# VachaLab/gorder

Hardware: AMD Instinct MI355X
Metric: trajectory frames/sec (higher is better)
Workload: dtype f32

## Files before the change

### gorder_amd/csrc/trajectory_driver.h

```cpp
#pragma once

#include <atomic>
#include <chrono>
#include <condition_variable>
#include <deque>
#include <mutex>
#include <thread>

#include "../../include/gorder_xtc.h"

namespace {

struct TrajSlot {
    float *h_xyz = nullptr, *h_box = nullptr, *h_time = nullptr;
    float *d_xyz = nullptr, *d_box = nullptr;
    uint8_t *h_blob = nullptr, *d_blob = nullptr;
    gorder_xtc_frame_t *h_frames = nullptr, *d_frames = nullptr;
    float *d_box_in = nullptr;
    uint32_t *d_stat = nullptr, *d_short = nullptr, *h_stat = nullptr, *h_short = nullptr;
    XtcCheckpoint *d_cp = nullptr;
    std::vector<int64_t> file_pos;
    std::vector<uint32_t> file_idx;
    uint32_t prefix_q16 = 65536;
    uint32_t kinds = 0;
    size_t moved = 0;
    uint64_t blob_bytes = 0;
    hipStream_t stream = nullptr;
    hipEvent_t staged = nullptr, copied = nullptr, computed = nullptr;
    bool copy_issued = false, compute_issued = false;
    uint32_t n = 0;
    std::vector<uint64_t> fidx;
};

struct TrajCache {
    static constexpr int kSlots = 4;
    TrajSlot slot[kSlots];
    bool dev = false, has_xtc = false;
    uint32_t batch = 0, n_stop = 0;
    size_t blob_cap = 0, xyz_bytes = 0;
    hipStream_t copy_stream = nullptr;
    unsigned long long *h_err = nullptr;
    float *h_fix = nullptr;
};

struct TrajPipe {
    static constexpr int kSlots = TrajCache::kSlots;
    TrajSlot *slot = nullptr;
    std::mutex mu;
    std::condition_variable cv;
    std::deque<int> free_q, filled_q;
    bool reader_done = false, stop = false;
    int reader_status = GORDER_XTC_OK;
    std::string reader_msg;
    double decode_s = 0.0, reader_stalled_s = 0.0, setup_s = 0.0;
    std::atomic<uint32_t> prefix_q16{65536};
    uint32_t reports = 0;
    bool alloc_failed = false;
};

double seconds_since(std::chrono::steady_clock::time_point t0) {
    return std::chrono::duration<double>(std::chrono::steady_clock::now() - t0).count();
}

void traj_cache_free(gorder_hip_handle *h) {
    TrajCache *c = static_cast<TrajCache *>(h->traj_cache);
    if (!c) return;
    for (TrajSlot &s : c->slot) {
        if (s.h_xyz) (void)hipHostFree(s.h_xyz);
        if (s.h_box) (void)hipHostFree(s.h_box);
        if (s.h_time) (void)hipHostFree(s.h_time);
        if (s.h_blob) (void)hipHostFree(s.h_blob);
        if (s.h_frames) (void)hipHostFree(s.h_frames);
        (void)hipFree(s.d_xyz);
        (void)hipFree(s.d_box);
        (void)hipFree(s.d_blob);
        (void)hipFree(s.d_frames);
        (void)hipFree(s.d_box_in);
        (void)hipFree(s.d_stat);
        (void)hipFree(s.d_short);
        (void)hipFree(s.d_cp);
        if (s.h_stat) (void)hipHostFree(s.h_stat);
        if (s.h_short) (void)hipHostFree(s.h_short);
        if (s.stream) (void)hipStreamDestroy(s.stream);
        if (s.staged) (void)hipEventDestroy(s.staged);
// ... 219 lines not shown
            {
                std::lock_guard<std::mutex> lk(pipe.mu);
                if (pipe.stop) return;
            }
            const auto t0 = std::chrono::steady_clock::now();
            const hipError_t e = alloc_slot(pipe.slot[k]);
            std::lock_guard<std::mutex> lk(pipe.mu);
            pipe.setup_s += seconds_since(t0);
            if (e != hipSuccess) { pipe.alloc_failed = true; return; }
            pipe.free_q.push_back(k);
            pipe.cv.notify_all();
        }
    });
    const double setup_s = seconds_since(t_start);

    gorder_xtc_pool *pool = nullptr;
    if (dev && gorder_xtc_pool_create(n_threads, &pool) != GORDER_XTC_OK) pool = nullptr;
    const char *forced_prefix = getenv("GORDER_HIP_PREFIX_Q16");
    const bool adapt_prefix = dev && has_xtc && !forced_prefix && !env_flag("GORDER_HIP_NO_PREFIX") && n_stop < n_file_atoms;
    if (dev && forced_prefix) pipe.prefix_q16.store((uint32_t)std::max(1l, std::min(65536l, atol(forced_prefix))));
    const bool verify = dev && has_xtc && (adapt_prefix || forced_prefix);
    const int device = h->device;
    std::thread reader([&, device]() {
        (void)hipSetDevice(device);
        uint64_t state = 0, analysed = shard_lo;
        double last_time = -INFINITY;
        uint32_t f = 0;
        gorder_xtc_reader *r = nullptr;
        bool done = shard_n == 0;
        uint32_t n_filled = 0;
        uint64_t to_skip = shard_lo, left = shard_n;
        auto give_up = [&](int st, const std::string &msg) {
            std::lock_guard<std::mutex> lk(pipe.mu);
            pipe.reader_status = st;
            pipe.reader_msg = msg;
            done = true;
        };
        while (!done) {
            int k = -1;
            {
                const auto t0 = std::chrono::steady_clock::now();
                std::unique_lock<std::mutex> lk(pipe.mu);
                pipe.cv.wait(lk, [&] { return pipe.stop || !pipe.free_q.empty(); });
                pipe.reader_stalled_s += seconds_since(t0);
                if (pipe.stop) break;
                k = pipe.free_q.front();
                pipe.free_q.pop_front();
            }
            TrajSlot &s = pipe.slot[k];
            const auto t_wait = std::chrono::steady_clock::now();
            if (s.copy_issued) (void)hipEventSynchronize(s.staged);
            const auto t1 = std::chrono::steady_clock::now();
            {
                std::lock_guard<std::mutex> lk(pipe.mu);
                pipe.reader_stalled_s += std::chrono::duration<double>(t1 - t_wait).count();
            }
            s.n = 0;
            s.blob_bytes = 0;
            uint32_t fill = batch;
            if (adapt_prefix && tr->batch_frames == 0 && f < tr->n_paths && file_is_xtc[f]) {
                if (n_filled == 0) fill = std::min(batch, 256u);
                else if (n_filled == 1) fill = std::min(batch, 1024u);
                else if (n_filled == 2) {
                    std::unique_lock<std::mutex> lk(pipe.mu);
                    pipe.cv.wait(lk, [&] { return pipe.stop || pipe.reports > 0; });
                }
            }
            s.prefix_q16 = pipe.prefix_q16.load();
            while (!done && s.n < fill) {
                if (left == 0) { done = true; break; }
                if (!r) {
                    if (f == tr->n_paths) { done = true; break; }
                    int st = gorder_xtc_open(tr->paths[f], tr->group, tr->n_group, &r);
                    if (st == GORDER_XTC_OK && gorder_xtc_n_atoms_out(r) != n_atoms) st = GORDER_XTC_ERR_ARGUMENT;
                    if (st != GORDER_XTC_OK) {
                        give_up(st, std::string("cannot read ") + tr->paths[f] +
                                        (st == GORDER_XTC_ERR_ARGUMENT ? ": atoms per frame differ from the tables" : ""));
                        break;
                    }
                }
                if (to_skip) {
                    const int64_t sk = gorder_xtc_skip_window(r, tr->begin_ps, tr->end_ps, tr->step, &state, &last_time, to_skip);
                    if (sk < 0) { give_up((int)sk, std::string("read error in ") + tr->paths[f]); break; }
                    to_skip -= (uint64_t)sk;
                    if (to_skip) {
                        gorder_xtc_close(r);
                        r = nullptr;
                        f++;
                        continue;
                    }
                }
                const uint64_t want = std::min<uint64_t>(fill - s.n, left);
                uint64_t used = 0;
                const int64_t got =
                    dev ? gorder_xtc_pack_window_ex(r, tr->begin_ps, tr->end_ps, tr->step, &state, &last_time,
                                                    s.h_blob + s.blob_bytes, blob_cap - s.blob_bytes, &used, s.h_frames + s.n,
                                                    s.h_box + 9u * (size_t)s.n, s.h_time + s.n, want, n_threads, pool,
                                                    s.prefix_q16, s.file_pos.data() + s.n)
                        : gorder_xtc_read_window_mt(r, tr->begin_ps, tr->end_ps, tr->step, &state, &last_time,
                                                    s.h_xyz + (size_t)s.n * n_atoms * 3u, s.h_box + 9u * (size_t)s.n,
                                                    s.h_time + s.n, want, n_threads);
                if (dev && got == GORDER_XTC_ERR_NO_SPACE) {
                    if (s.n > 0) break;
                    give_up(GORDER_XTC_ERR_ARGUMENT, std::string("a single frame of ") + tr->paths[f] + " does not fit the staging blob");
                    break;
                }
                if (got < 0) {
                    give_up((int)got, std::string("read error in ") + tr->paths[f]);
                    break;
                }
                if (got == 0) {
                    gorder_xtc_close(r);
                    r = nullptr;
                    f++;
                    continue;
                }
                if (dev) {
                    for (int64_t q = 0; q < got; q++) {
                        s.h_frames[s.n + (size_t)q].offset += s.blob_bytes;
                        s.file_idx[s.n + (size_t)q] = f;
                    }
                    s.blob_bytes += used;
                }
                s.n += (uint32_t)got;
                left -= (uint64_t)got;
            }
            if (pool) {
                const int cst = gorder_xtc_pool_wait(pool);
                if (cst != GORDER_XTC_OK && !done) give_up(cst, "read error while copying the compressed blocks");
                else if (cst != GORDER_XTC_OK) { std::lock_guard<std::mutex> lk(pipe.mu); if (pipe.reader_status == GORDER_XTC_OK) { pipe.reader_status = cst; pipe.reader_msg = "read error while copying the compressed blocks"; } }
            }
            const double dt = seconds_since(t1);
            std::lock_guard<std::mutex> lk(pipe.mu);
            pipe.decode_s += dt;
            if (s.n == 0 || pipe.reader_status != GORDER_XTC_OK) {
                pipe.free_q.push_front(k);
                break;
            }
            if (dev && (xtc_table_kinds(s.h_frames, s.n) & kXtcTableXtc)) n_filled++;
            s.fidx.resize((size_t)s.n);
            for (uint32_t q = 0; q < s.n; q++) s.fidx[q] = tr->first_frame_index + (analysed + q) * tr->step;
            analysed += s.n;
            pipe.filled_q.push_back(k);
            pipe.cv.notify_all();
        }
        if (r) gorder_xtc_close(r);
        std::lock_guard<std::mutex> lk(pipe.mu);
        pipe.reader_done = true;
        pipe.cv.notify_all();
    });

    int status = GORDER_OK;
    uint64_t frames = 0, batches = 0, bytes = 0, frames_fixed = 0;
    double starved_s = 0.0;
    std::string hip_msg;
    uint32_t need_q16 = 0;
    auto stage_a = [&](int k) {
        TrajSlot &s = pipe.slot[k];
        const size_t nx = (size_t)s.n * n_atoms * 3u * sizeof(float), nb = (size_t)s.n * 9u * sizeof(float);
        hipError_t e = hipSuccess;
        const hipStream_t feed = dev ? s.stream : copy_stream;
        if (s.compute_issued && !dev) e = hipStreamWaitEvent(feed, s.computed, 0);
        s.moved = nb;
        if (dev) {
            const size_t nf = (size_t)s.n * sizeof(gorder_xtc_frame_t);
            s.moved += (size_t)s.blob_bytes + nf;
            if (e == hipSuccess) e = hipMemsetAsync(s.d_stat, 0, 2 * sizeof(uint32_t), feed);
            if (e == hipSuccess) e = hipMemsetAsync(s.d_stat + 2, 0xff, 2 * sizeof(uint32_t), feed);
            if (e == hipSuccess) e = hipMemcpyAsync(s.d_blob, s.h_blob, (size_t)s.blob_bytes, hipMemcpyHostToDevice, feed);
            if (e == hipSuccess) e = hipMemcpyAsync(s.d_frames, s.h_frames, nf, hipMemcpyHostToDevice, feed);
            if (e == hipSuccess) e = hipMemcpyAsync(s.d_box_in, s.h_box, nb, hipMemcpyHostToDevice, feed);
            if (e == hipSuccess) e = hipEventRecord(s.staged, feed);
            if (e == hipSuccess && s.compute_issued) e = hipStreamWaitEvent(feed, s.computed, 0);
            if (e == hipSuccess) e = hipMemcpyAsync(s.d_box, s.d_box_in, nb, hipMemcpyDeviceToDevice, feed);
            s.kinds = xtc_table_kinds(s.h_frames, s.n);
            if (e == hipSuccess && status == GORDER_OK)
                status = xtc_decode_on(h, feed, s.d_blob, s.blob_bytes, s.d_frames, s.n, n_file_atoms, d_slot_of, n_stop,
// ... 91 lines not shown
            while (!pipe.filled_q.empty()) {
                fresh.push_back(pipe.filled_q.front());
                pipe.filled_q.pop_front();
            }
            finished = pipe.reader_done && fresh.empty() && decoding.empty();
        }
        if (finished) break;
        for (int k : fresh) {
            if (!go) break;
            stage_a(k);
            if (verify) decoding.push_back(k);
            else go = stage_b(k);
        }
        bool any = !fresh.empty();
        while (go && !decoding.empty() &&
               (status != GORDER_OK || hipEventQuery(pipe.slot[decoding.front()].copied) == hipSuccess)) {
            const int front = decoding.front();
            decoding.pop_front();
            go = stage_b(front);
            any = true;
        }
        if (go && !any && !decoding.empty()) {
            std::unique_lock<std::mutex> lk(pipe.mu);
            pipe.cv.wait_for(lk, std::chrono::microseconds(100), [&] { return !pipe.filled_q.empty(); });
        }
    }
    {
        std::lock_guard<std::mutex> lk(pipe.mu);
        pipe.stop = true;
        pipe.cv.notify_all();
    }
    reader.join();
    allocator.join();
    if (pool) gorder_xtc_pool_destroy(pool);
    (void)hipStreamSynchronize(copy_stream);
    for (int k = 0; k < TrajPipe::kSlots; k++)
        if (pipe.slot[k].stream) (void)hipStreamSynchronize(pipe.slot[k].stream);
    const int sync_status = gorder_hip_synchronize(h);
    if (status == GORDER_OK) status = sync_status;
    else if (!hip_msg.empty()) h->err_msg = hip_msg;
    if (status == GORDER_OK && pipe.reader_status != GORDER_XTC_OK) {
        status = pipe.reader_status == GORDER_XTC_ERR_FORMAT ? GORDER_ERR_TRAJECTORY_FORMAT : GORDER_ERR_INVALID_ARGUMENT;
        h->err_msg = pipe.reader_msg + " (reader status " + std::to_string(pipe.reader_status) + ")";
    }
    if (stats) {
        stats->n_frames = frames;
        stats->n_batches = batches;
        stats->bytes_h2d = bytes;
        stats->seconds_total = seconds_since(t_start);
        stats->seconds_decode = pipe.decode_s;
        stats->seconds_reader_stalled = pipe.reader_stalled_s;
        stats->seconds_gpu_starved = starved_s;
        stats->batch_frames = batch;
        stats->decoder_threads = n_threads;
        stats->device_decode = dev ? 1u : 0u;
        stats->frames_decoded_by_host = (uint32_t)std::min<uint64_t>(frames_fixed, UINT32_MAX);
        stats->seconds_setup = setup_s + pipe.setup_s;
        stats->shard_first = shard_lo;
        stats->shard_frames_total = tr->shard_count > 1 ? shard_total : frames;
    }
    cleanup();
    if (pipe.alloc_failed) traj_cache_free(h);
#undef TRAJ_TRY
    return status;
}
```

### gorder_amd/csrc/xtc_reader.cpp

```cpp
#include <algorithm>
#include <climits>
#include <cmath>
#include <cstdint>
#include <cstdio>
#include <cstring>
#include <string>
#include <string>
#include <atomic>
#include <chrono>
#include <condition_variable>
#include <deque>
#include <functional>
#include <memory>
#include <mutex>
#include <thread>
#include <immintrin.h>
#include <sys/mman.h>
#include <sys/stat.h>
#include <unistd.h>
#include <vector>

#include "../../include/gorder_xtc.h"

namespace {

const int kMagicInts[] = {
    0,       0,       0,       0,       0,       0,       0,       0,       0,       8,        10,       12,
    16,      20,      25,      32,      40,      50,      64,      80,      101,     128,      161,      203,
    256,     322,     406,     512,     645,     812,     1024,    1290,    1625,    2048,     2580,     3250,
    4096,    5060,    6501,    8192,    10321,   13003,   16384,   20642,   26007,   32768,    41285,    52015,
    65536,   82570,   104031,  131072,  165140,  208063,  262144,  330280,  416127,  524287,   660561,   832255,
    1048576, 1321122, 1664510, 2097152, 2642245, 3329021, 4194304, 5284491, 6658042, 8388607,  10568983, 13316085,
    16777216};
constexpr int kFirstIdx = 9;
constexpr int kLastIdx = (int)(sizeof(kMagicInts) / sizeof(kMagicInts[0]));

struct BitReader {
    const uint8_t *p;
    size_t n, bitpos = 0;
    bool overrun = false;

    static uint64_t load_be64(const uint8_t *q) {
        uint64_t w;
        memcpy(&w, q, 8);
        return __builtin_bswap64(w);
    }
    uint64_t bits57(int nbits) {
        if (nbits == 0) return 0;
// ... 104 lines not shown
    memcpy(&f, &u, 4);
    return f;
}

double bed(const uint8_t *p) {
    uint64_t u = 0;
    for (int k = 0; k < 8; k++) u = (u << 8) | p[k];
    double d;
    memcpy(&d, &u, 8);
    return d;
}

}

struct FileMap {
    const uint8_t *base = nullptr;
    size_t size = 0;
    ~FileMap() { if (base) munmap(const_cast<uint8_t *>(base), size); }
};

struct gorder_xtc_reader {
    std::string path;
    FILE *fp = nullptr;
    bool trr = false;
    bool gro = false;
    uint32_t natoms = 0;
    std::vector<uint32_t> group;
    std::vector<int32_t> slot_of;
    uint32_t n_needed = 0;
    std::vector<uint8_t> buf;
    std::vector<int> ints;
    std::shared_ptr<struct FileMap> map;
    bool map_tried = false;
};

namespace {

bool read_exact(FILE *fp, void *dst, size_t n) { return fread(dst, 1, n, fp) == n; }

int decode_ints(gorder_xtc_reader *r, const int minint[3], const int maxint[3], int smallidx, const uint8_t *data,
                size_t nbytes) {
    const uint32_t natoms = r->natoms;
    r->ints.resize((size_t)natoms * 3);
    uint32_t sizeint[3];
    int bitsizeint[3] = {0, 0, 0};
    for (int k = 0; k < 3; k++) {
        const int64_t s = (int64_t)maxint[k] - (int64_t)minint[k] + 1;
        if (s <= 0 || s > 0xffffffffll) return GORDER_XTC_ERR_FORMAT;
        sizeint[k] = (uint32_t)s;
    }
    int bitsize;
    if ((sizeint[0] | sizeint[1] | sizeint[2]) > 0xffffff) {
        for (int k = 0; k < 3; k++) bitsizeint[k] = size_of_int(sizeint[k]);
        bitsize = 0;
    } else {
        bitsize = size_of_ints(sizeint);
    }
    if (smallidx < kFirstIdx || smallidx >= kLastIdx) return GORDER_XTC_ERR_FORMAT;
    int smaller = kMagicInts[smallidx > kFirstIdx ? smallidx - 1 : kFirstIdx] / 2;
    int smallnum = kMagicInts[smallidx] / 2;
    uint32_t sizesmall[3] = {(uint32_t)kMagicInts[smallidx], (uint32_t)kMagicInts[smallidx], (uint32_t)kMagicInts[smallidx]};
    const uint64_t recip_big[3] = {reciprocal_of(sizeint[0]), reciprocal_of(sizeint[1]), reciprocal_of(sizeint[2])};
    uint64_t recip_small[3] = {kMagicRecips.r[smallidx], kMagicRecips.r[smallidx], kMagicRecips.r[smallidx]};

    BitReader br{data, nbytes};
    int *out = r->ints.data();
// ... 619 lines not shown
        *last_time = (double)t;
        if (t < begin_ps) continue;
        if (end_ps >= 0.0f && t > end_ps) { fseek(r->fp, 0, SEEK_END); break; }
        const uint64_t k = (*state)++;
        if (k % step != 0) continue;
        offsets.push_back(pos);
    }
    const size_t nout = gorder_xtc_n_atoms_out(r), n = offsets.size();
    const uint32_t nt = (uint32_t)std::min<size_t>(n_threads, std::max<size_t>(n, 1));
    std::vector<int> status(nt, GORDER_XTC_OK);
    std::vector<std::thread> pool;
    for (uint32_t w = 0; w < nt; w++)
        pool.emplace_back([&, w]() {
            gorder_xtc_reader *mine = nullptr;
            int st = gorder_xtc_open(r->path.c_str(), r->group.empty() ? nullptr : r->group.data(), (uint32_t)r->group.size(), &mine);
            for (size_t i = w; st == GORDER_XTC_OK && i < n; i += nt) {
                if (fseek(mine->fp, offsets[i], SEEK_SET) != 0) { st = GORDER_XTC_ERR_FORMAT; break; }
                float t = 0.0f;
                st = gorder_xtc_next(mine, xyz + i * nout * 3, box9 + i * 9, nullptr, &t, nullptr);
                if (st == GORDER_XTC_OK && time_ps) time_ps[i] = t;
            }
            gorder_xtc_close(mine);
            status[w] = st;
        });
    for (auto &th : pool) th.join();
    for (int st : status)
        if (st != GORDER_XTC_OK) return st == GORDER_XTC_EOF ? GORDER_XTC_ERR_FORMAT : st;
    return (int64_t)n;
}

}

struct gorder_xtc_pool {
    std::vector<std::thread> workers;
    std::mutex mu;
    std::condition_variable cv_work, cv_idle;
    std::deque<std::function<int()>> jobs;
    size_t running = 0;
    int status = GORDER_XTC_OK;
    bool stop = false;
    void loop() {
        for (;;) {
            std::function<int()> job;
            {
                std::unique_lock<std::mutex> lk(mu);
                cv_work.wait(lk, [&] { return stop || !jobs.empty(); });
                if (jobs.empty()) return;
                job = std::move(jobs.front());
                jobs.pop_front();
                running++;
            }
            const int st = job();
            std::lock_guard<std::mutex> lk(mu);
            if (st != GORDER_XTC_OK && status == GORDER_XTC_OK) status = st;
            running--;
            if (jobs.empty() && running == 0) cv_idle.notify_all();
        }
    }
};

extern "C" {

int gorder_xtc_pool_create(uint32_t n_threads, gorder_xtc_pool **out) {
    if (!out) return GORDER_XTC_ERR_ARGUMENT;
    gorder_xtc_pool *p = new gorder_xtc_pool();
    for (uint32_t w = 0; w < std::max(1u, n_threads); w++) p->workers.emplace_back([p] { p->loop(); });
    *out = p;
    return GORDER_XTC_OK;
}
int gorder_xtc_pool_wait(gorder_xtc_pool *p) {
    if (!p) return GORDER_XTC_ERR_ARGUMENT;
    std::unique_lock<std::mutex> lk(p->mu);
    p->cv_idle.wait(lk, [&] { return p->jobs.empty() && p->running == 0; });
    const int st = p->status;
    p->status = GORDER_XTC_OK;
    return st;
}
void gorder_xtc_pool_destroy(gorder_xtc_pool *p) {
    if (!p) return;
    {
        std::lock_guard<std::mutex> lk(p->mu);
        p->stop = true;
    }
    p->cv_work.notify_all();
    for (auto &t : p->workers) t.join();
    delete p;
}


int gorder_xtc_probe(const char *path, uint32_t *n_atoms, uint64_t *file_bytes, uint32_t *first_frame_bytes) {
    if (!path) return GORDER_XTC_ERR_ARGUMENT;
    FILE *fp = fopen(path, "rb");
    if (!fp) return GORDER_XTC_ERR_OPEN;
    uint8_t head[92];
    const size_t got = fread(head, 1, sizeof(head), fp);
    if (file_bytes) {
        *file_bytes = 0;
        if (fseeko(fp, 0, SEEK_END) == 0) *file_bytes = (uint64_t)ftello(fp);
    }
    fclose(fp);
    if (got < 8) return GORDER_XTC_ERR_FORMAT;
    if (be32(head) != 1995u) return 0;
    const uint32_t na = be32(head + 4);
    if (n_atoms) *n_atoms = na;
    if (first_frame_bytes) {
        *first_frame_bytes = 0;
        if (na <= 9 && got >= 56) *first_frame_bytes = 56u + 12u * na;
        else if (na > 9 && got == sizeof(head)) *first_frame_bytes = 92u + ((be32(head + 88) + 3u) & ~3u);
    }
    return 1;
}
int gorder_xtc_probe_format(const char *path, int *format, uint32_t *n_atoms, uint64_t *file_bytes, uint32_t *first_frame_bytes) {
    if (!path || !format) return GORDER_XTC_ERR_ARGUMENT;
    *format = GORDER_XTC_FORMAT_OTHER;
    if (n_atoms) *n_atoms = 0;
    if (first_frame_bytes) *first_frame_bytes = 0;
    const int xtc = gorder_xtc_probe(path, n_atoms, file_bytes, first_frame_bytes);
    if (xtc < 0) return xtc;
// ... 20 lines not shown
        pos += (off_t)(hlen + body);
    }
    fclose(fp);
    return GORDER_XTC_OK;
}
int gorder_xtc_is_xtc(const gorder_xtc_reader *r) { return (r && !r->trr && !r->gro) ? 1 : 0; }
int gorder_xtc_can_pack(const gorder_xtc_reader *r) { return (r && !r->gro) ? 1 : 0; }
uint32_t gorder_xtc_n_atoms_needed(const gorder_xtc_reader *r) {
    return r ? (r->n_needed ? std::min(r->n_needed, r->natoms) : r->natoms) : 0;
}

}

namespace {
struct PackSrc { off_t pos; uint32_t n; uint64_t dst; };
__attribute__((target("avx2"))) void stream_copy_avx2(uint8_t *dst, const uint8_t *src, size_t n) {
    size_t i = 0;
    for (; i + 128 <= n; i += 128) {
        const __m256i a = _mm256_loadu_si256((const __m256i *)(src + i)), b = _mm256_loadu_si256((const __m256i *)(src + i + 32));
        const __m256i c = _mm256_loadu_si256((const __m256i *)(src + i + 64)), d = _mm256_loadu_si256((const __m256i *)(src + i + 96));
        _mm256_stream_si256((__m256i *)(dst + i), a);
        _mm256_stream_si256((__m256i *)(dst + i + 32), b);
        _mm256_stream_si256((__m256i *)(dst + i + 64), c);
        _mm256_stream_si256((__m256i *)(dst + i + 96), d);
    }
    if (i < n) memcpy(dst + i, src + i, n - i);
    _mm_sfence();
}
bool have_avx2() {
    static const bool yes = __builtin_cpu_supports("avx2");
    return yes;
}
int pack_copy(int fd, const FileMap *map, const PackSrc *src, size_t i0, size_t i1, uint8_t *blob) {
    const bool stream = map && map->base && have_avx2() && !getenv("GORDER_XTC_PREAD");
    for (size_t i = i0; i < i1; i++) {
        uint8_t *dst = blob + src[i].dst;
        size_t done = 0;
        if (stream && ((uintptr_t)dst & 31u) == 0 && (size_t)src[i].pos + src[i].n <= map->size) {
            stream_copy_avx2(dst, map->base + src[i].pos, src[i].n);
            done = src[i].n;
        }
        while (done < src[i].n) {
            const ssize_t g = pread(fd, dst + done, src[i].n - done, src[i].pos + (off_t)done);
            if (g <= 0) return GORDER_XTC_ERR_FORMAT;
            done += (size_t)g;
        }
        const size_t end = (size_t)((((uint64_t)src[i].n + 63u) & ~63ull) + 64u);
        memset(dst + src[i].n, 0, end - src[i].n);
    }
    return GORDER_XTC_OK;
}

int64_t pack_window_impl(gorder_xtc_reader *r, float begin_ps, float end_ps, uint32_t step, uint64_t *state,
                         double *last_time, uint8_t *blob, uint64_t blob_capacity, uint64_t *blob_bytes,
                         gorder_xtc_frame_t *frames, float *box9, float *time_ps, uint64_t capacity,
                         uint32_t n_threads, gorder_xtc_pool *pool, uint32_t prefix_q16 = 65536u, int64_t *file_pos = nullptr) {
    if (!r || !r->fp || r->gro || !state || !last_time || !blob || !blob_bytes || !frames || !box9 || step == 0)
        return GORDER_XTC_ERR_ARGUMENT;
    *blob_bytes = 0;
    const auto t_scan0 = std::chrono::steady_clock::now();
    std::vector<PackSrc> src;
    uint64_t used = 0;
    const uint32_t natoms = r->natoms;
    const int fd = fileno(r->fp);
    off_t pos = (off_t)ftello(r->fp);
    bool to_end = false;
    const uint64_t state_at_entry = *state;
    const double last_time_at_entry = *last_time;
    struct stat sb;
    const off_t file_end = fstat(fd, &sb) == 0 && S_ISREG(sb.st_mode) ? sb.st_size : (off_t)-1;
    if (!r->map_tried) {
        r->map_tried = true;
        if (file_end > 0) {
            void *m = mmap(nullptr, (size_t)file_end, PROT_READ, MAP_SHARED, fd, 0);
            if (m != MAP_FAILED) {
                (void)madvise(m, (size_t)file_end, MADV_SEQUENTIAL);
                r->map = std::make_shared<FileMap>();
                r->map->base = static_cast<const uint8_t *>(m);
                r->map->size = (size_t)file_end;
            }
        }
    }
    if (r->map && (getenv("GORDER_XTC_PREAD") || (file_end >= 0 && (size_t)file_end < r->map->size))) r->map.reset();
    const FileMap *map = r->map.get();
    auto fetch = [&](off_t at, uint8_t *dst, size_t n) -> ssize_t {
        if (map && map->base && at >= 0 && (size_t)at + n <= map->size) {
            memcpy(dst, map->base + at, n);
            return (ssize_t)n;
        }
        return pread(fd, dst, n, at);
    };
    const uint32_t n_stop = gorder_xtc_n_atoms_needed(r);
    while (src.size() < capacity) {
        const off_t pos0 = pos;
        uint8_t head[56 + 36];
        float t;
        float trr_box[9] = {0.0f, 0.0f, 0.0f, 0.0f, 0.0f, 0.0f, 0.0f, 0.0f, 0.0f};
        gorder_xtc_frame_t fr{};
        uint32_t block = 0;
        uint32_t copy = 0;
        off_t pos_block;
        if (r->trr) {
            uint8_t th[kTrrHeadMax];
            const ssize_t got = fetch(pos0, th, sizeof(th));
            if (got < 0) return GORDER_XTC_ERR_FORMAT;
            TrrHeader h{};
            size_t hlen = 0;
            const int st = trr_parse_header(th, (size_t)got, h, &hlen);
            if (st == GORDER_XTC_EOF) break;
            if (st != GORDER_XTC_OK || h.natoms != natoms) return GORDER_XTC_ERR_FORMAT;
            const off_t before_x = (off_t)hlen + (off_t)h.sizes[0] + h.sizes[1] + h.sizes[2] + h.sizes[3] + h.sizes[4] + h.sizes[5] + h.sizes[6];
            pos = pos0 + before_x + (off_t)h.sizes[7] + h.sizes[8] + h.sizes[9];
            if (h.sizes[7] == 0) continue;
            if (h.sizes[7] != (uint64_t)natoms * 3u * h.real_size) return GORDER_XTC_ERR_FORMAT;
            pos_block = pos0 + before_x;
            block = h.sizes[7];
            if (file_end >= 0 && pos_block + (off_t)block > file_end) return GORDER_XTC_ERR_FORMAT;
            if (h.sizes[2]) {
                uint8_t b[72];
                if (h.sizes[2] > sizeof(b) || fetch(pos0 + (off_t)hlen + h.sizes[0] + h.sizes[1], b, h.sizes[2]) != (ssize_t)h.sizes[2])
                    return GORDER_XTC_ERR_FORMAT;
                for (int q = 0; q < 9; q++) trr_box[q] = h.real_size == 4 ? bef(b + 4 * q) : (float)bed(b + 8 * q);
            }
            t = (float)h.t;
            fr.kind = h.real_size == 4 ? 4u : 8u;
            fr.n_bytes = copy = n_stop * 3u * h.real_size;
// ... 19 lines not shown
                }
                if ((fr.sizeint[0] | fr.sizeint[1] | fr.sizeint[2]) > 0xffffff) {
                    fr.bitsize = 0;
                    for (int k = 0; k < 3; k++) fr.bitsizeint |= (uint32_t)size_of_int(fr.sizeint[k]) << (8 * k);
                } else {
                    fr.bitsize = (uint32_t)size_of_ints(fr.sizeint);
                }
                fr.recip1 = reciprocal_of(fr.sizeint[1]);
                fr.recip2 = reciprocal_of(fr.sizeint[2]);
                fr.smallidx = (int32_t)be32(h2 + 28);
                if (fr.smallidx < kFirstIdx || fr.smallidx >= kLastIdx) return GORDER_XTC_ERR_FORMAT;
                fr.inv_precision = 1.0f / bef(h2);
                block = (uint32_t)(((size_t)be32(h2 + 32) + 3) & ~(size_t)3);
                fr.n_bytes = block;
                pos_block = pos0 + (off_t)sizeof(head);
            }
            copy = block;
            if (prefix_q16 < 65536u && natoms > 9) {
                const uint64_t c = (((uint64_t)block * prefix_q16 >> 16) + 2048u + 3u) & ~3ull;
                if (c < block) { copy = (uint32_t)c; fr.kind |= 2u; fr.n_bytes = copy; }
            }
            pos = pos_block + (off_t)block;
            if (file_end >= 0 && pos > file_end) return GORDER_XTC_ERR_FORMAT;
        }
        if ((double)t == *last_time) continue;
        const double time_before = *last_time;
        *last_time = (double)t;
        if (t < begin_ps) continue;
        if (end_ps >= 0.0f && t > end_ps) { to_end = true; break; }
        const uint64_t k = (*state)++;
        if (k % step != 0) continue;
        const uint64_t need = (((uint64_t)copy + 63u) & ~63ull) + 64u;
        if (used + need > blob_capacity) {
            if (src.empty()) {
                *state = state_at_entry;
                *last_time = last_time_at_entry;
                return GORDER_XTC_ERR_NO_SPACE;
            }
            (*state)--;
            *last_time = time_before;
            pos = pos0;
            break;
        }
        const size_t i = src.size();
        fr.offset = used;
        used += need;
        frames[i] = fr;
        for (int q = 0; q < 9; q++) box9[9 * i + q] = r->trr ? trr_box[q] : bef(head + 16 + 4 * q);
        if (time_ps) time_ps[i] = t;
        if (file_pos) file_pos[i] = (int64_t)pos0;
        src.push_back({pos_block, copy, fr.offset});
    }
    if (to_end ? fseek(r->fp, 0, SEEK_END) != 0 : fseeko(r->fp, pos, SEEK_SET) != 0) return GORDER_XTC_ERR_FORMAT;
    const size_t n = src.size();
    if (n == 0) return 0;
    const auto t_copy0 = std::chrono::steady_clock::now();
    if (pool) {
        const size_t nj = std::min<size_t>(pool->workers.size(), n);
        auto shared = std::make_shared<std::vector<PackSrc>>(std::move(src));
        const int fd2 = dup(fd);
        if (fd2 < 0) return GORDER_XTC_ERR_OPEN;
        auto left = std::make_shared<std::atomic<size_t>>(nj);
        std::shared_ptr<FileMap> keep = r->map;
        {
            std::lock_guard<std::mutex> lk(pool->mu);
            for (size_t w = 0; w < nj; w++) {
                const size_t i0 = n * w / nj, i1 = n * (w + 1) / nj;
                pool->jobs.emplace_back([shared, fd2, left, i0, i1, blob, keep]() {
                    const int st = pack_copy(fd2, keep.get(), shared->data(), i0, i1, blob);
                    if (left->fetch_sub(1) == 1) close(fd2);
                    return st;
                });
            }
        }
        pool->cv_work.notify_all();
        *blob_bytes = used;
        return (int64_t)n;
    }
    const uint32_t nt = (uint32_t)std::min<size_t>(std::max(1u, n_threads), n);
    std::vector<int> status(nt, GORDER_XTC_OK);
    auto work = [&](uint32_t w) { status[w] = pack_copy(fd, map, src.data(), n * w / nt, n * (w + 1) / nt, blob); };
    if (nt == 1) {
        work(0);
    } else {
        std::vector<std::thread> threads;
        for (uint32_t w = 0; w < nt; w++) threads.emplace_back(work, w);
        for (auto &th : threads) th.join();
    }
    for (int st : status)
        if (st != GORDER_XTC_OK) return st;
    if (getenv("GORDER_XTC_PACK_TIMING")) {
        const auto t1 = std::chrono::steady_clock::now();
        fprintf(stderr, "pack_window: %zu frames, scan %.3f ms, copy %.3f ms (%u threads, %.1f MB)\n", n,
                std::chrono::duration<double, std::milli>(t_copy0 - t_scan0).count(),
                std::chrono::duration<double, std::milli>(t1 - t_copy0).count(), nt, used / 1e6);
    }
    *blob_bytes = used;
    return (int64_t)n;
}
}

extern "C" {

int64_t gorder_xtc_pack_window(gorder_xtc_reader *r, float begin_ps, float end_ps, uint32_t step, uint64_t *state,
                               double *last_time, uint8_t *blob, uint64_t blob_capacity, uint64_t *blob_bytes,
                               gorder_xtc_frame_t *frames, float *box9, float *time_ps, uint64_t capacity,
                               uint32_t n_threads) {
    return pack_window_impl(r, begin_ps, end_ps, step, state, last_time, blob, blob_capacity, blob_bytes, frames, box9,
                            time_ps, capacity, n_threads, nullptr);
}

int64_t gorder_xtc_pack_window_ex(gorder_xtc_reader *r, float begin_ps, float end_ps, uint32_t step, uint64_t *state,
                                  double *last_time, uint8_t *blob, uint64_t blob_capacity, uint64_t *blob_bytes,
                                  gorder_xtc_frame_t *frames, float *box9, float *time_ps, uint64_t capacity,
// ... 22 lines not shown
```

### gorder_amd/xtc.py

```python
from __future__ import annotations

import ctypes as C
from typing import Optional, Sequence

import numpy as np

from .abi import load_library

_bound = False


def _lib():
    global _bound
    lib = load_library()
    if not _bound:
        vp = C.c_void_p
        lib.gorder_xtc_open.argtypes = [C.c_char_p, vp, C.c_uint32, C.POINTER(vp)]
        lib.gorder_xtc_close.argtypes = [vp]
        lib.gorder_xtc_close.restype = None
        lib.gorder_xtc_n_atoms_file.argtypes = [vp]
        lib.gorder_xtc_n_atoms_file.restype = C.c_uint32
        lib.gorder_xtc_n_atoms_out.argtypes = [vp]
        lib.gorder_xtc_n_atoms_out.restype = C.c_uint32
        lib.gorder_xtc_next.argtypes = [vp, vp, vp, C.POINTER(C.c_int64), C.POINTER(C.c_float), C.POINTER(C.c_float)]
        lib.gorder_xtc_read_window.argtypes = [vp, C.c_float, C.c_float, C.c_uint32, C.POINTER(C.c_uint64),
                                               C.POINTER(C.c_double), vp, vp, vp, C.c_uint64]
        lib.gorder_xtc_read_window.restype = C.c_int64
        lib.gorder_xtc_read_window_mt.argtypes = [vp, C.c_float, C.c_float, C.c_uint32, C.POINTER(C.c_uint64),
                                                  C.POINTER(C.c_double), vp, vp, vp, C.c_uint64, C.c_uint32]
        lib.gorder_xtc_read_window_mt.restype = C.c_int64
        lib.gorder_xtc_pack_window.argtypes = [vp, C.c_float, C.c_float, C.c_uint32, C.POINTER(C.c_uint64),
                                               C.POINTER(C.c_double), vp, C.c_uint64, C.POINTER(C.c_uint64), vp, vp, vp,
                                               C.c_uint64, C.c_uint32]
        lib.gorder_xtc_pack_window.restype = C.c_int64
        lib.gorder_xtc_skip_window.argtypes = [vp, C.c_float, C.c_float, C.c_uint32, C.POINTER(C.c_uint64),
                                               C.POINTER(C.c_double), C.c_uint64]
        lib.gorder_xtc_skip_window.restype = C.c_int64
        lib.gorder_xtc_pool_create.argtypes = [C.c_uint32, C.POINTER(vp)]
        lib.gorder_xtc_pool_wait.argtypes = [vp]
        lib.gorder_xtc_pool_destroy.argtypes = [vp]
        lib.gorder_xtc_pool_destroy.restype = None
        lib.gorder_xtc_pack_window_pool.argtypes = [vp, C.c_float, C.c_float, C.c_uint32, C.POINTER(C.c_uint64),
                                                    C.POINTER(C.c_double), vp, C.c_uint64, C.POINTER(C.c_uint64), vp, vp, vp,
                                                    C.c_uint64, vp]
        lib.gorder_xtc_pack_window_pool.restype = C.c_int64
        lib.gorder_xtc_pack_window_ex.argtypes = [vp, C.c_float, C.c_float, C.c_uint32, C.POINTER(C.c_uint64),
                                                  C.POINTER(C.c_double), vp, C.c_uint64, C.POINTER(C.c_uint64), vp, vp, vp,
                                                  C.c_uint64, C.c_uint32, vp, C.c_uint32, vp]
        lib.gorder_xtc_pack_window_ex.restype = C.c_int64
        lib.gorder_xtc_is_xtc.argtypes = [vp]
        lib.gorder_xtc_can_pack.argtypes = [vp]
        lib.gorder_xtc_probe_format.argtypes = [C.c_char_p, C.POINTER(C.c_int), C.POINTER(C.c_uint32), C.POINTER(C.c_uint64),
                                                C.POINTER(C.c_uint32)]
        lib.gorder_xtc_read_at.argtypes = [vp, C.c_int64, vp, vp]
        lib.gorder_xtc_probe.argtypes = [C.c_char_p, C.POINTER(C.c_uint32), C.POINTER(C.c_uint64), C.POINTER(C.c_uint32)]
        lib.gorder_xtc_n_atoms_needed.argtypes = [vp]
        lib.gorder_xtc_n_atoms_needed.restype = C.c_uint32
        lib.gorder_xtc_writer_open.argtypes = [C.c_char_p, C.c_uint32, C.c_float, C.POINTER(vp)]
        lib.gorder_xtc_writer_add.argtypes = [vp, vp, vp, C.c_int64, C.c_float]
        lib.gorder_xtc_writer_close.argtypes = [vp]
        lib.gorder_xtc_writer_close.restype = None
        _bound = True
    return lib


def write_trajectory(path: str, xyz: np.ndarray, box: np.ndarray, times: Optional[Sequence[float]] = None,
                     precision: float = 1000.0, append_to=None):
    lib = _lib()
    xyz = np.ascontiguousarray(xyz, dtype=np.float32)
    box = np.ascontiguousarray(box, dtype=np.float32).reshape(xyz.shape[0], 9)
    if times is None:
        times = np.arange(xyz.shape[0], dtype=np.float32)
    w = C.c_void_p()
    st = lib.gorder_xtc_writer_open(path.encode(), xyz.shape[1], precision, C.byref(w))
# ... 189 lines not shown
```

### include/gorder_xtc.h

```cpp
#ifndef GORDER_XTC_H
#define GORDER_XTC_H

#include <stddef.h>
#include <stdint.h>

#ifdef __cplusplus
extern "C" {
#endif

typedef struct gorder_xtc_reader gorder_xtc_reader;

typedef enum {
    GORDER_XTC_OK = 0,
    GORDER_XTC_EOF = 1,
    GORDER_XTC_ERR_OPEN = -1,
    GORDER_XTC_ERR_FORMAT = -2,
    GORDER_XTC_ERR_ARGUMENT = -3,
    GORDER_XTC_ERR_NO_SPACE = -4
} gorder_xtc_status_t;

int gorder_xtc_open(const char *path, const uint32_t *group, uint32_t n_group, gorder_xtc_reader **out);
void gorder_xtc_close(gorder_xtc_reader *r);
uint32_t gorder_xtc_n_atoms_file(const gorder_xtc_reader *r);
uint32_t gorder_xtc_n_atoms_out(const gorder_xtc_reader *r);
// ... 3 lines not shown

int64_t gorder_xtc_read_window(gorder_xtc_reader *r, float begin_ps, float end_ps, uint32_t step,
                               uint64_t *state, double *last_time, float *xyz, float *box9, float *time_ps,
                               uint64_t capacity);

int64_t gorder_xtc_skip_window(gorder_xtc_reader *r, float begin_ps, float end_ps, uint32_t step, uint64_t *state,
                               double *last_time, uint64_t max_frames);

int64_t gorder_xtc_read_window_mt(gorder_xtc_reader *r, float begin_ps, float end_ps, uint32_t step,
                                  uint64_t *state, double *last_time, float *xyz, float *box9, float *time_ps,
                                  uint64_t capacity, uint32_t n_threads);

typedef struct {
    uint64_t offset;
    uint64_t recip1, recip2;
    uint32_t n_bytes;
    uint32_t kind;
    int32_t minint[3];
    uint32_t sizeint[3];
    int32_t smallidx;
    float inv_precision;
    uint32_t bitsize;
    uint32_t bitsizeint;
} gorder_xtc_frame_t;

int64_t gorder_xtc_pack_window(gorder_xtc_reader *r, float begin_ps, float end_ps, uint32_t step, uint64_t *state,
                               double *last_time, uint8_t *blob, uint64_t blob_capacity, uint64_t *blob_bytes,
                               gorder_xtc_frame_t *frames, float *box9, float *time_ps, uint64_t capacity,
                               uint32_t n_threads);
typedef struct gorder_xtc_pool gorder_xtc_pool;
int gorder_xtc_pool_create(uint32_t n_threads, gorder_xtc_pool **out);
int gorder_xtc_pool_wait(gorder_xtc_pool *pool);
void gorder_xtc_pool_destroy(gorder_xtc_pool *pool);
int64_t gorder_xtc_pack_window_pool(gorder_xtc_reader *r, float begin_ps, float end_ps, uint32_t step, uint64_t *state,
                                    double *last_time, uint8_t *blob, uint64_t blob_capacity, uint64_t *blob_bytes,
                                    gorder_xtc_frame_t *frames, float *box9, float *time_ps, uint64_t capacity,
                                    gorder_xtc_pool *pool);

int64_t gorder_xtc_pack_window_ex(gorder_xtc_reader *r, float begin_ps, float end_ps, uint32_t step, uint64_t *state,
                                  double *last_time, uint8_t *blob, uint64_t blob_capacity, uint64_t *blob_bytes,
                                  gorder_xtc_frame_t *frames, float *box9, float *time_ps, uint64_t capacity,
                                  uint32_t n_threads, gorder_xtc_pool *pool, uint32_t prefix_q16, int64_t *file_pos);
int gorder_xtc_read_at(gorder_xtc_reader *r, int64_t file_pos, float *xyz, float *box9);

int gorder_xtc_probe(const char *path, uint32_t *n_atoms, uint64_t *file_bytes, uint32_t *first_frame_bytes);
enum { GORDER_XTC_FORMAT_OTHER = 0, GORDER_XTC_FORMAT_XTC = 1, GORDER_XTC_FORMAT_TRR = 2 };
int gorder_xtc_probe_format(const char *path, int *format, uint32_t *n_atoms, uint64_t *file_bytes,
                            uint32_t *first_frame_bytes);
int gorder_xtc_is_xtc(const gorder_xtc_reader *r);
int gorder_xtc_can_pack(const gorder_xtc_reader *r);
uint32_t gorder_xtc_n_atoms_needed(const gorder_xtc_reader *r);

typedef struct gorder_xtc_writer gorder_xtc_writer;
int gorder_xtc_writer_open(const char *path, uint32_t n_atoms, float precision, gorder_xtc_writer **out);
int gorder_xtc_writer_add(gorder_xtc_writer *w, const float *xyz, const float *box9, int64_t step, float time_ps);
void gorder_xtc_writer_close(gorder_xtc_writer *w);

#ifdef __cplusplus
}
#endif
#endif
```

Baseline: 20.67 million.

## Overlap XTC block copying with scanning via grouped pool jobs and publisher thread

The pack step now flushes copy jobs to the worker pool incrementally, every fixed number of frames and in byte-bounded chunks, so copying starts while the header scan is still running. Jobs are tagged with a per-batch group, and a separate publisher thread waits for each group before handing the slot to the GPU side. This lets the reader start scanning the next batch instead of blocking on the whole pool. It adds more threads, locking and error-propagation paths (copy_failed), plus optional timing instrumentation, at the risk of extra synchronisation overhead and races.

```diff
diff --git a/gorder_amd/csrc/trajectory_driver.h b/gorder_amd/csrc/trajectory_driver.h
--- a/gorder_amd/csrc/trajectory_driver.h
+++ b/gorder_amd/csrc/trajectory_driver.h
@@ -50,6 +50,9 @@
     std::condition_variable cv;
     std::deque<int> free_q, filled_q;
     bool reader_done = false, stop = false;
+    struct Scanned { int k; uint64_t group; std::chrono::steady_clock::time_point t_begin; bool good; };
+    std::deque<Scanned> scanned_q;
+    bool copy_failed = false;
     int reader_status = GORDER_XTC_OK;
     std::string reader_msg;
     double decode_s = 0.0, reader_stalled_s = 0.0, setup_s = 0.0;
@@ -335,18 +338,58 @@
         uint64_t to_skip = shard_lo, left = shard_n;
         auto give_up = [&](int st, const std::string &msg) {
             std::lock_guard<std::mutex> lk(pipe.mu);
-            pipe.reader_status = st;
-            pipe.reader_msg = msg;
+            if (!pipe.copy_failed) {
+                pipe.reader_status = st;
+                pipe.reader_msg = msg;
+            }
             done = true;
         };
+        std::chrono::steady_clock::time_point busy_until = t_start;
+        auto publish = [&](int k, std::chrono::steady_clock::time_point t_begin, bool good) {
+            const auto t_end = std::chrono::steady_clock::now();
+            pipe.decode_s += std::max(0.0, std::chrono::duration<double>(t_end - std::max(t_begin, busy_until)).count());
+            busy_until = std::max(busy_until, t_end);
+            if (!good || pipe.copy_failed) {
+                pipe.free_q.push_front(k);
+                return false;
+            }
+            pipe.filled_q.push_back(k);
+            pipe.cv.notify_all();
+            return true;
+        };
+        std::thread publisher;
+        if (pool) publisher = std::thread([&]() {
+            for (bool open = true;;) {
+                TrajPipe::Scanned sc;
+                {
+                    std::unique_lock<std::mutex> lk(pipe.mu);
+                    pipe.cv.wait(lk, [&] { return !pipe.scanned_q.empty(); });
+                    sc = pipe.scanned_q.front();
+                    pipe.scanned_q.pop_front();
+                }
+                if (sc.k < 0) return;
+                const int cst = gorder_xtc_pool_wait_group(pool, sc.group);
+                std::lock_guard<std::mutex> lk(pipe.mu);
+                if (cst != GORDER_XTC_OK && !pipe.copy_failed) {
+                    pipe.copy_failed = true;
+                    if (sc.good || pipe.reader_status == GORDER_XTC_OK) {
+                        pipe.reader_status = cst;
+                        pipe.reader_msg = "read error while copying the compressed blocks";
+                    }
+                    pipe.cv.notify_all();
+                }
+                if (!open) pipe.free_q.push_front(sc.k);
+                else open = publish(sc.k, sc.t_begin, sc.good);
+            }
+        });
         while (!done) {
             int k = -1;
             {
                 const auto t0 = std::chrono::steady_clock::now();
                 std::unique_lock<std::mutex> lk(pipe.mu);
-                pipe.cv.wait(lk, [&] { return pipe.stop || !pipe.free_q.empty(); });
+                pipe.cv.wait(lk, [&] { return pipe.stop || pipe.copy_failed || !pipe.free_q.empty(); });
                 pipe.reader_stalled_s += seconds_since(t0);
-                if (pipe.stop) break;
+                if (pipe.stop || pipe.copy_failed) break;
                 k = pipe.free_q.front();
                 pipe.free_q.pop_front();
             }
@@ -366,10 +409,11 @@
                 else if (n_filled == 1) fill = std::min(batch, 1024u);
                 else if (n_filled == 2) {
                     std::unique_lock<std::mutex> lk(pipe.mu);
-                    pipe.cv.wait(lk, [&] { return pipe.stop || pipe.reports > 0; });
+                    pipe.cv.wait(lk, [&] { return pipe.stop || pipe.copy_failed || pipe.reports > 0; });
                 }
             }
             s.prefix_q16 = pipe.prefix_q16.load();
+            const uint64_t group = pool ? gorder_xtc_pool_group_begin(pool) : 0;
             while (!done && s.n < fill) {
                 if (left == 0) { done = true; break; }
                 if (!r) {
@@ -428,24 +472,33 @@
                 s.n += (uint32_t)got;
                 left -= (uint64_t)got;
             }
+            bool good;
+            {
+                std::lock_guard<std::mutex> lk(pipe.mu);
+                good = s.n > 0 && pipe.reader_status == GORDER_XTC_OK;
+            }
+            if (good) {
+                if (dev && (xtc_table_kinds(s.h_frames, s.n) & kXtcTableXtc)) n_filled++;
+                s.fidx.resize((size_t)s.n);
+                for (uint32_t q = 0; q < s.n; q++) s.fidx[q] = tr->first_frame_index + (analysed + q) * tr->step;
+                analysed += s.n;
+            }
+            std::lock_guard<std::mutex> lk(pipe.mu);
             if (pool) {
-                const int cst = gorder_xtc_pool_wait(pool);
-                if (cst != GORDER_XTC_OK && !done) give_up(cst, "read error while copying the compressed blocks");
-                else if (cst != GORDER_XTC_OK) { std::lock_guard<std::mutex> lk(pipe.mu); if (pipe.reader_status == GORDER_XTC_OK) { pipe.reader_status = cst; pipe.reader_msg = "read error while copying the compressed blocks"; } }
-            }
-            const double dt = seconds_since(t1);
-            std::lock_guard<std::mutex> lk(pipe.mu);
-            pipe.decode_s += dt;
-            if (s.n == 0 || pipe.reader_status != GORDER_XTC_OK) {
-                pipe.free_q.push_front(k);
+                pipe.scanned_q.push_back({k, group, t1, good});
+                pipe.cv.notify_all();
+                if (!good) break;
+            } else if (!publish(k, t1, good)) {
                 break;
             }
-            if (dev && (xtc_table_kinds(s.h_frames, s.n) & kXtcTableXtc)) n_filled++;
-            s.fidx.resize((size_t)s.n);
-            for (uint32_t q = 0; q < s.n; q++) s.fidx[q] = tr->first_frame_index + (analysed + q) * tr->step;
-            analysed += s.n;
-            pipe.filled_q.push_back(k);
-            pipe.cv.notify_all();
+        }
+        if (publisher.joinable()) {
+            {
+                std::lock_guard<std::mutex> lk(pipe.mu);
+                pipe.scanned_q.push_back({-1, 0, t_start, false});
+                pipe.cv.notify_all();
+            }
+            publisher.join();
         }
         if (r) gorder_xtc_close(r);
         std::lock_guard<std::mutex> lk(pipe.mu);
@@ -603,7 +656,10 @@
     }
     reader.join();
     allocator.join();
-    if (pool) gorder_xtc_pool_destroy(pool);
+    if (pool) {
+        (void)gorder_xtc_pool_wait(pool);
+        gorder_xtc_pool_destroy(pool);
+    }
     (void)hipStreamSynchronize(copy_stream);
     for (int k = 0; k < TrajPipe::kSlots; k++)
         if (pipe.slot[k].stream) (void)hipStreamSynchronize(pipe.slot[k].stream);
diff --git a/gorder_amd/csrc/xtc_reader.cpp b/gorder_amd/csrc/xtc_reader.cpp
--- a/gorder_amd/csrc/xtc_reader.cpp
+++ b/gorder_amd/csrc/xtc_reader.cpp
@@ -14,6 +14,7 @@
 #include <memory>
 #include <mutex>
 #include <thread>
+#include <unordered_map>
 #include <immintrin.h>
 #include <sys/mman.h>
 #include <sys/stat.h>
@@ -184,6 +185,7 @@
     std::vector<int> ints;
     std::shared_ptr<struct FileMap> map;
     bool map_tried = false;
+    bool pread_only = false, avx2 = false;
 };
 
 namespace {
@@ -869,29 +871,58 @@
 }
 
 struct gorder_xtc_pool {
+    struct Job { std::function<int()> run; uint64_t group; };
+    struct Group { size_t pending = 0; int status = GORDER_XTC_OK; };
     std::vector<std::thread> workers;
     std::mutex mu;
-    std::condition_variable cv_work, cv_idle;
-    std::deque<std::function<int()>> jobs;
+    std::condition_variable cv_work, cv_done;
+    std::deque<Job> jobs;
     size_t running = 0;
     int status = GORDER_XTC_OK;
     bool stop = false;
+    std::unordered_map<uint64_t, Group> groups;
+    uint64_t current = 0, next_group = 1;
+    uint32_t flush_frames = 256;
+    uint64_t job_bytes = (uint64_t)2 << 20;
+    bool timing = false, scanning = false;
+    size_t n_idle = 0;
+    double scan_s = 0.0, job_s = 0.0, idle_scan_s = 0.0;
+    std::chrono::steady_clock::time_point last_event;
+    void account() {
+        const auto now = std::chrono::steady_clock::now();
+        if (scanning) idle_scan_s += (double)n_idle * std::chrono::duration<double>(now - last_event).count();
+        last_event = now;
+    }
+    void scan_mark(bool begin) {
+        if (!timing) return;
+        std::lock_guard<std::mutex> lk(mu);
+        account();
+        scanning = begin;
+    }
     void loop() {
         for (;;) {
-            std::function<int()> job;
+            Job job;
             {
                 std::unique_lock<std::mutex> lk(mu);
+                if (timing) { account(); n_idle++; }
                 cv_work.wait(lk, [&] { return stop || !jobs.empty(); });
+                if (timing) { account(); n_idle--; }
                 if (jobs.empty()) return;
                 job = std::move(jobs.front());
                 jobs.pop_front();
                 running++;
             }
-            const int st = job();
+            const auto t0 = std::chrono::steady_clock::now();
+            const int st = job.run();
+            job.run = nullptr;
             std::lock_guard<std::mutex> lk(mu);
+            if (timing) job_s += std::chrono::duration<double>(std::chrono::steady_clock::now() - t0).count();
             if (st != GORDER_XTC_OK && status == GORDER_XTC_OK) status = st;
+            Group &g = groups[job.group];
+            if (st != GORDER_XTC_OK && g.status == GORDER_XTC_OK) g.status = st;
+            g.pending--;
             running--;
-            if (jobs.empty() && running == 0) cv_idle.notify_all();
+            if (g.pending == 0 || (jobs.empty() && running == 0)) cv_done.notify_all();
         }
     }
 };
@@ -901,14 +932,41 @@
 int gorder_xtc_pool_create(uint32_t n_threads, gorder_xtc_pool **out) {
     if (!out) return GORDER_XTC_ERR_ARGUMENT;
     gorder_xtc_pool *p = new gorder_xtc_pool();
+    p->timing = getenv("GORDER_XTC_PACK_TIMING") != nullptr;
+    p->last_event = std::chrono::steady_clock::now();
+    p->groups[0];
     for (uint32_t w = 0; w < std::max(1u, n_threads); w++) p->workers.emplace_back([p] { p->loop(); });
     *out = p;
     return GORDER_XTC_OK;
 }
+int gorder_xtc_pool_set_granularity(gorder_xtc_pool *p, uint32_t flush_frames, uint64_t job_bytes) {
+    if (!p) return GORDER_XTC_ERR_ARGUMENT;
+    std::lock_guard<std::mutex> lk(p->mu);
+    p->flush_frames = flush_frames ? flush_frames : 256u;
+    p->job_bytes = job_bytes ? job_bytes : (uint64_t)2 << 20;
+    return GORDER_XTC_OK;
+}
+uint64_t gorder_xtc_pool_group_begin(gorder_xtc_pool *p) {
+    if (!p) return 0;
+    std::lock_guard<std::mutex> lk(p->mu);
+    p->current = p->next_group++;
+    p->groups[p->current];
+    return p->current;
+}
+int gorder_xtc_pool_wait_group(gorder_xtc_pool *p, uint64_t id) {
+    if (!p) return GORDER_XTC_ERR_ARGUMENT;
+    std::unique_lock<std::mutex> lk(p->mu);
+    if (p->groups.find(id) == p->groups.end()) return GORDER_XTC_ERR_ARGUMENT;
+    p->cv_done.wait(lk, [&] { return p->groups[id].pending == 0; });
+    const int st = p->groups[id].status;
+    if (id != 0 && id != p->current) p->groups.erase(id);
+    else p->groups[id].status = GORDER_XTC_OK;
+    return st;
+}
 int gorder_xtc_pool_wait(gorder_xtc_pool *p) {
     if (!p) return GORDER_XTC_ERR_ARGUMENT;
     std::unique_lock<std::mutex> lk(p->mu);
-    p->cv_idle.wait(lk, [&] { return p->jobs.empty() && p->running == 0; });
+    p->cv_done.wait(lk, [&] { return p->jobs.empty() && p->running == 0; });
     const int st = p->status;
     p->status = GORDER_XTC_OK;
     return st;
@@ -921,6 +979,9 @@
     }
     p->cv_work.notify_all();
     for (auto &t : p->workers) t.join();
+    if (p->timing)
+        fprintf(stderr, "pack_pool: scan %.6f s, jobs %.6f s, workers idle during scan %.6f s (%zu workers)\n", p->scan_s,
+                p->job_s, p->idle_scan_s, p->workers.size());
     delete p;
 }
 
@@ -1007,7 +1068,7 @@
     return yes;
 }
 int pack_copy(int fd, const FileMap *map, const PackSrc *src, size_t i0, size_t i1, uint8_t *blob) {
-    const bool stream = map && map->base && have_avx2() && !getenv("GORDER_XTC_PREAD");
+    const bool stream = map && map->base;
     for (size_t i = i0; i < i1; i++) {
         uint8_t *dst = blob + src[i].dst;
         size_t done = 0;
@@ -1034,6 +1095,16 @@
         return GORDER_XTC_ERR_ARGUMENT;
     *blob_bytes = 0;
     const auto t_scan0 = std::chrono::steady_clock::now();
+    struct ScanMark {
+        gorder_xtc_pool *p;
+        std::chrono::steady_clock::time_point t0;
+        ~ScanMark() {
+            if (!p || !p->timing) return;
+            p->scan_mark(false);
+            p->scan_s += std::chrono::duration<double>(std::chrono::steady_clock::now() - t0).count();
+        }
+    } scan_mark{pool, t_scan0};
+    if (pool) pool->scan_mark(true);
     std::vector<PackSrc> src;
     uint64_t used = 0;
     const uint32_t natoms = r->natoms;
@@ -1046,6 +1117,8 @@
     const off_t file_end = fstat(fd, &sb) == 0 && S_ISREG(sb.st_mode) ? sb.st_size : (off_t)-1;
     if (!r->map_tried) {
         r->map_tried = true;
+        r->pread_only = getenv("GORDER_XTC_PREAD") != nullptr;
+        r->avx2 = have_avx2();
         if (file_end > 0) {
             void *m = mmap(nullptr, (size_t)file_end, PROT_READ, MAP_SHARED, fd, 0);
             if (m != MAP_FAILED) {
@@ -1056,8 +1129,9 @@
             }
         }
     }
-    if (r->map && (getenv("GORDER_XTC_PREAD") || (file_end >= 0 && (size_t)file_end < r->map->size))) r->map.reset();
+    if (r->map && (r->pread_only || (file_end >= 0 && (size_t)file_end < r->map->size))) r->map.reset();
     const FileMap *map = r->map.get();
+    const FileMap *copy_map = r->avx2 ? map : nullptr;
     auto fetch = [&](off_t at, uint8_t *dst, size_t n) -> ssize_t {
         if (map && map->base && at >= 0 && (size_t)at + n <= map->size) {
             memcpy(dst, map->base + at, n);
@@ -1066,7 +1140,51 @@
         return pread(fd, dst, n, at);
     };
     const uint32_t n_stop = gorder_xtc_n_atoms_needed(r);
-    while (src.size() < capacity) {
+    struct PackCall {
+        int fd = -1;
+        std::shared_ptr<FileMap> keep;
+        const FileMap *map = nullptr;
+        ~PackCall() { if (fd >= 0) close(fd); }
+    };
+    std::shared_ptr<PackCall> call;
+    size_t n_total = 0;
+    uint32_t flush_frames = 0;
+    uint64_t job_bytes = 0;
+    if (pool) {
+        std::lock_guard<std::mutex> lk(pool->mu);
+        flush_frames = pool->flush_frames;
+        job_bytes = pool->job_bytes;
+    }
+    auto flush = [&]() -> int {
+        if (src.empty()) return GORDER_XTC_OK;
+        if (!call) {
+            call = std::make_shared<PackCall>();
+            call->fd = dup(fd);
+            if (call->fd < 0) return GORDER_XTC_ERR_OPEN;
+            call->keep = r->map;
+            call->map = copy_map;
+        }
+        auto shared = std::make_shared<std::vector<PackSrc>>(std::move(src));
+        src.clear();
+        const size_t n = shared->size();
+        {
+            std::lock_guard<std::mutex> lk(pool->mu);
+            const uint64_t group = pool->current;
+            for (size_t i0 = 0; i0 < n;) {
+                size_t i1 = i0;
+                for (uint64_t bytes = 0; i1 < n && bytes < job_bytes; i1++) bytes += (*shared)[i1].n;
+                std::shared_ptr<PackCall> c = call;
+                pool->jobs.push_back({[shared, c, i0, i1, blob]() {
+                                          return pack_copy(c->fd, c->map, shared->data(), i0, i1, blob);
+                                      }, group});
+                pool->groups[group].pending++;
+                i0 = i1;
+            }
+        }
+        pool->cv_work.notify_all();
+        return GORDER_XTC_OK;
+    };
+    while (n_total < capacity) {
         const off_t pos0 = pos;
         uint8_t head[56 + 36];
         float t;
@@ -1152,7 +1270,7 @@
         if (k % step != 0) continue;
         const uint64_t need = (((uint64_t)copy + 63u) & ~63ull) + 64u;
         if (used + need > blob_capacity) {
-            if (src.empty()) {
+            if (n_total == 0) {
                 *state = state_at_entry;
                 *last_time = last_time_at_entry;
                 return GORDER_XTC_ERR_NO_SPACE;
@@ -1162,7 +1280,7 @@
             pos = pos0;
             break;
         }
-        const size_t i = src.size();
+        const size_t i = n_total++;
         fr.offset = used;
         used += need;
         frames[i] = fr;
@@ -1170,36 +1288,24 @@
         if (time_ps) time_ps[i] = t;
         if (file_pos) file_pos[i] = (int64_t)pos0;
         src.push_back({pos_block, copy, fr.offset});
+        if (pool && src.size() >= flush_frames) {
+            const int st = flush();
+            if (st != GORDER_XTC_OK) return st;
+        }
     }
     if (to_end ? fseek(r->fp, 0, SEEK_END) != 0 : fseeko(r->fp, pos, SEEK_SET) != 0) return GORDER_XTC_ERR_FORMAT;
-    const size_t n = src.size();
+    const size_t n = n_total;
     if (n == 0) return 0;
     const auto t_copy0 = std::chrono::steady_clock::now();
     if (pool) {
-        const size_t nj = std::min<size_t>(pool->workers.size(), n);
-        auto shared = std::make_shared<std::vector<PackSrc>>(std::move(src));
-        const int fd2 = dup(fd);
-        if (fd2 < 0) return GORDER_XTC_ERR_OPEN;
-        auto left = std::make_shared<std::atomic<size_t>>(nj);
-        std::shared_ptr<FileMap> keep = r->map;
-        {
-            std::lock_guard<std::mutex> lk(pool->mu);
-            for (size_t w = 0; w < nj; w++) {
-                const size_t i0 = n * w / nj, i1 = n * (w + 1) / nj;
-                pool->jobs.emplace_back([shared, fd2, left, i0, i1, blob, keep]() {
-                    const int st = pack_copy(fd2, keep.get(), shared->data(), i0, i1, blob);
-                    if (left->fetch_sub(1) == 1) close(fd2);
-                    return st;
-                });
-            }
-        }
-        pool->cv_work.notify_all();
+        const int st = flush();
+        if (st != GORDER_XTC_OK) return st;
         *blob_bytes = used;
         return (int64_t)n;
     }
     const uint32_t nt = (uint32_t)std::min<size_t>(std::max(1u, n_threads), n);
     std::vector<int> status(nt, GORDER_XTC_OK);
-    auto work = [&](uint32_t w) { status[w] = pack_copy(fd, map, src.data(), n * w / nt, n * (w + 1) / nt, blob); };
+    auto work = [&](uint32_t w) { status[w] = pack_copy(fd, copy_map, src.data(), n * w / nt, n * (w + 1) / nt, blob); };
     if (nt == 1) {
         work(0);
     } else {
diff --git a/gorder_amd/xtc.py b/gorder_amd/xtc.py
--- a/gorder_amd/xtc.py
+++ b/gorder_amd/xtc.py
@@ -40,6 +40,11 @@
         lib.gorder_xtc_pool_wait.argtypes = [vp]
         lib.gorder_xtc_pool_destroy.argtypes = [vp]
         lib.gorder_xtc_pool_destroy.restype = None
+        if hasattr(lib, "gorder_xtc_pool_group_begin"):
+            lib.gorder_xtc_pool_set_granularity.argtypes = [vp, C.c_uint32, C.c_uint64]
+            lib.gorder_xtc_pool_group_begin.argtypes = [vp]
+            lib.gorder_xtc_pool_group_begin.restype = C.c_uint64
+            lib.gorder_xtc_pool_wait_group.argtypes = [vp, C.c_uint64]
         lib.gorder_xtc_pack_window_pool.argtypes = [vp, C.c_float, C.c_float, C.c_uint32, C.POINTER(C.c_uint64),
                                                     C.POINTER(C.c_double), vp, C.c_uint64, C.POINTER(C.c_uint64), vp, vp, vp,
                                                     C.c_uint64, vp]
diff --git a/include/gorder_xtc.h b/include/gorder_xtc.h
--- a/include/gorder_xtc.h
+++ b/include/gorder_xtc.h
@@ -59,6 +59,9 @@
 int gorder_xtc_pool_create(uint32_t n_threads, gorder_xtc_pool **out);
 int gorder_xtc_pool_wait(gorder_xtc_pool *pool);
 void gorder_xtc_pool_destroy(gorder_xtc_pool *pool);
+int gorder_xtc_pool_set_granularity(gorder_xtc_pool *pool, uint32_t flush_frames, uint64_t job_bytes);
+uint64_t gorder_xtc_pool_group_begin(gorder_xtc_pool *pool);
+int gorder_xtc_pool_wait_group(gorder_xtc_pool *pool, uint64_t group);
 int64_t gorder_xtc_pack_window_pool(gorder_xtc_reader *r, float begin_ps, float end_ps, uint32_t step, uint64_t *state,
                                     double *last_time, uint8_t *blob, uint64_t blob_capacity, uint64_t *blob_bytes,
                                     gorder_xtc_frame_t *frames, float *box9, float *time_ps, uint64_t capacity,
```

Result: no change. 20.77 million, median of 2 (+0.5%).
